# felipeagc/sycl-ray-tracer

Hardware: AMD Instinct MI355X
Metric: Mrays/s (higher is better)
Workload: dtype f32

## Files before the change

include/rt_mi355x.h:

```cpp
#ifndef RT_MI355X_H
#define RT_MI355X_H

#include <stddef.h>
#include <stdint.h>

#ifdef __cplusplus
extern "C" {
#endif

#define RT_ABI_VERSION 8

typedef enum rt_status {
    RT_OK = 0,
    RT_ERR_INVALID = -1,
    RT_ERR_NO_DEVICE = -2,
    RT_ERR_HIP = -3,
    RT_ERR_OOM = -4,
    RT_ERR_UNSUPPORTED = -5
} rt_status;

#define RT_TEX_SIZE 512u
#define RT_TEX_CHANNELS 4u
#define RT_TEX_MAX_LAYERS 128u

// ... 253 lines not shown
                    int want_device_u8);
int rt_frame_gather_begin(rt_comm* c, rt_renderer* const* renderers, int want_f32, int want_u8);
int rt_comm_wait(rt_comm* c, float* rgba_f32, uint8_t* rgba_u8);
int rt_comm_size(const rt_comm* c);
const void* rt_comm_frame_f32(const rt_comm* c);
const void* rt_comm_frame_u8(const rt_comm* c);

int rt_probe_xorshift(int device, uint32_t seed, uint32_t n, float* out, uint32_t* state_out);
int rt_probe_half_roundtrip(int device, uint32_t n, const float* in, float* out,
                            uint16_t* bits_out);
int rt_probe_scatter(rt_scene* scene, uint32_t material, uint32_t n, const float* dir,
                     const float* normal, const float* uv, const uint32_t* seed, uint8_t* ok,
                     float* out_dir, float* out_att, uint32_t* seed_out);

int rt_probe_rounding(int device, uint64_t* mismatches);

const char* rt_last_error(void);
int rt_abi_version(void);
int rt_device_count(void);

#ifdef __cplusplus
}
#endif
#endif
```

sycl-ray-tracer_amd/csrc/rt_device.h:

```cpp
#pragma once
#include <hip/hip_runtime.h>

#include "../../include/rt_mi355x.h"
#include "rt_types.h"

namespace rt {

#define RT_DEV __device__ __forceinline__

struct f3 {
    float x, y, z;
};
RT_DEV f3 mk3(float x, float y, float z) { return f3{x, y, z}; }
RT_DEV f3 operator+(f3 a, f3 b) { return mk3(a.x + b.x, a.y + b.y, a.z + b.z); }
RT_DEV f3 operator-(f3 a, f3 b) { return mk3(a.x - b.x, a.y - b.y, a.z - b.z); }
RT_DEV f3 operator-(f3 a) { return mk3(-a.x, -a.y, -a.z); }
RT_DEV f3 operator*(f3 a, f3 b) { return mk3(a.x * b.x, a.y * b.y, a.z * b.z); }
RT_DEV f3 operator*(float s, f3 a) { return mk3(s * a.x, s * a.y, s * a.z); }
RT_DEV f3 operator*(f3 a, float s) { return mk3(a.x * s, a.y * s, a.z * s); }
RT_DEV float dot3(f3 a, f3 b) { return (a.x * b.x + a.y * b.y) + a.z * b.z; }
RT_DEV f3 cross3(f3 a, f3 b) {
    return mk3(a.y * b.z - a.z * b.y, a.z * b.x - a.x * b.z, a.x * b.y - a.y * b.x);
}
RT_DEV float rcp_rn(float x) {
// ... 6 lines not shown
    return 1.0f / x;
}
RT_DEV float inv_sqrt2(float x) {
    const bool ok = __float_as_uint(x) - 0x0C800000u < 0x73000000u;
    if (__builtin_expect(__builtin_amdgcn_ballot_w64(!ok) == 0ull, 1)) {
        const float r = __builtin_amdgcn_rsqf(x);
        float g = x * r, h = 0.5f * r;
        const float e = __builtin_fmaf(-h, g, 0.5f);
        g = __builtin_fmaf(g, e, g), h = __builtin_fmaf(h, e, h);
        const float s = __builtin_fmaf(__builtin_fmaf(-g, g, x), h, g);
        const float y = __builtin_amdgcn_rcpf(s);
        return __builtin_fmaf(__builtin_fmaf(-s, y, 1.0f), y, y);
    }
    return 1.0f / __builtin_sqrtf(x);
}
RT_DEV f3 normalize3(f3 a) {
    const float inv = inv_sqrt2(dot3(a, a));
    return mk3(a.x * inv, a.y * inv, a.z * inv);
}
RT_DEV float clamp01(float x) { return __builtin_fminf(__builtin_fmaxf(x, 0.0f), 1.0f); }

RT_DEV uint16_t f2h(float f) {
    asm("" : "+v"(f));
    _Float16 h = (_Float16)f;
    return __builtin_bit_cast(uint16_t, h);
}
RT_DEV float h2f(uint16_t b) { return (float)__builtin_bit_cast(_Float16, b); }

RT_DEV float rng_next(uint32_t& a) {
    uint32_t x = a;
    x ^= x << 13;
    x ^= x >> 17;
    x ^= x << 5;
    a = x;
    return (float)x * (1.0f / 4294967296.0f);
}
RT_DEV float rng_range(uint32_t& a, float mn, float mx) { return mn + (mx - mn) * rng_next(a); }
RT_DEV f3 rng_unit_vector(uint32_t& a) {
    float x = rng_range(a, -1.0f, 1.0f);
    float y = rng_range(a, -1.0f, 1.0f);
    float z = rng_range(a, -1.0f, 1.0f);
    return normalize3(mk3(x, y, z));
// ... 170 lines not shown
}
RT_DEV int32_t sel(lmask m, int32_t a, int32_t b) { return (int32_t)sel(m, (uint32_t)a, (uint32_t)b); }

struct TravSigns {
    lmask nx, ny, nz;
};

RT_DEV float ub0(uint32_t w) { return (float)(w & 0xffu); }
RT_DEV float ub1(uint32_t w) { return (float)((w >> 8) & 0xffu); }
RT_DEV float ub2(uint32_t w) { return (float)((w >> 16) & 0xffu); }
RT_DEV float ub3(uint32_t w) { return (float)(w >> 24); }

struct WaveStats {
    uint32_t inner_steps = 0, inner_lanes = 0, leaf_steps = 0, leaf_lanes = 0;
    uint32_t shade_rounds = 0, shade_lanes = 0, live_lane_steps = 0, top_lanes = 0;
};
RT_DEV TravSigns trav_signs(const Trav& T) { return TravSigns{lanes(T.ix < 0.0f), lanes(T.iy < 0.0f), lanes(T.iz < 0.0f)}; }
RT_DEV void trav_inner(const SceneDev& S, Trav& T, const TravStack& stack, const TopTree& top, const TravSigns& sg) {
    const float inf = __builtin_huge_valf();
    float k0, k1, k2, k3;
    u32x4 w0, w1, w2, chw;
    if (T.cur < top.count * 64) {
        const uint32_t o = (uint32_t)T.cur >> 2;
        w0 = *(lds_u32x4*)(size_t)((uint32_t)(size_t)top.w0 + o), w1 = *(lds_u32x4*)(size_t)((uint32_t)(size_t)top.w1 + o);
        w2 = *(lds_u32x4*)(size_t)((uint32_t)(size_t)top.w2 + o), chw = *(lds_u32x4*)(size_t)((uint32_t)(size_t)top.ch + o);
    } else {
        asm volatile("global_load_dwordx4 %0, %4, %5\n\t"
                     "global_load_dwordx4 %1, %4, %5 offset:16\n\t"
                     "global_load_dwordx4 %2, %4, %5 offset:32\n\t"
                     "global_load_dwordx4 %3, %4, %5 offset:48"
// ... 95 lines not shown
}

RT_DEV Hit intersect(const SceneDev& S, f3 o, f3 d, const TravStack& stack, const TopTree& top) {
    Trav T;
    trav_begin(T, o, d, stack);
    const TravSigns sg = trav_signs(T);
    while (trav_step_wave(S, T, stack, top, sg)) {}
    return T.best;
}

RT_DEV bool near_zero3(f3 e) {
    const float s = 1e-8f;
    return (__builtin_fabsf(e.x) < s) && (__builtin_fabsf(e.y) < s) && (__builtin_fabsf(e.z) < s);
}
RT_DEV float length_squared3(f3 v) {
    float l = __builtin_sqrtf(dot3(v, v));
    return l * l;
}
RT_DEV f3 reflect3(f3 v, f3 n) { return v - (2.0f * dot3(v, n)) * n; }
RT_DEV f3 refract3(f3 uv, f3 n, float etai_over_etat) {
    float cos_theta = __builtin_fminf(dot3(-uv, n), 1.0f);
    f3 r_out_perp = etai_over_etat * (uv + cos_theta * n);
    f3 r_out_parallel = (-__builtin_sqrtf(__builtin_fabsf(1.0f - length_squared3(r_out_perp)))) * n;
    return r_out_perp + r_out_parallel;
}
RT_DEV float schlick(float cosine, float ref_idx) {
    float r0 = (1.0f - ref_idx) / (1.0f + ref_idx);
    r0 = r0 * r0;
    float x = 1.0f - cosine;
    float x2 = x * x;
    float x5 = (x2 * x2) * x;
    return r0 + (1.0f - r0) * x5;
}
RT_DEV float unorm8_to_float(uint32_t b) {
    const float x = (float)b, r = 1.0f / 255.0f;
    const float q = x * r;
    return __builtin_fmaf(__builtin_fmaf(-q, 255.0f, x), r, q);
}

RT_DEV bool albedo_is_texture(const MatRec& m) { return (m.type == RT_MAT_DIFFUSE || m.type == RT_MAT_METALLIC) && m.tex_kind != RT_TEX_COLOR; }
RT_DEV uint32_t albedo_fetch(const SceneDev& S, const MatRec& m, float u, float v) {
    float fu = u - __builtin_floorf(u);
    float fv = v - __builtin_floorf(v);
// ... 7 lines not shown
    return mk3(unorm8_to_float(texel & 0xffu), unorm8_to_float((texel >> 8) & 0xffu), unorm8_to_float((texel >> 16) & 0xffu));
}
RT_DEV f3 albedo(const SceneDev& S, const MatRec& m, float u, float v) {
    if (m.tex_kind == RT_TEX_COLOR) return mk3(m.color[0], m.color[1], m.color[2]);
    float fu = u - __builtin_floorf(u);
    float fv = v - __builtin_floorf(v);
    int iu = (int)__builtin_floorf(fu * 512.0f);
    int iv = (int)__builtin_floorf(fv * 512.0f);
    iu = iu < 0 ? 0 : (iu > 511 ? 511 : iu);
    iv = iv < 0 ? 0 : (iv > 511 ? 511 : iv);
    const uint32_t texel = *reinterpret_cast<const uint32_t*>(
        S.tex + (((size_t)m.tex_layer * 512u + (size_t)iv) * 512u + (size_t)iu) * 4u);
    return mk3(unorm8_to_float(texel & 0xffu), unorm8_to_float((texel >> 8) & 0xffu), unorm8_to_float((texel >> 16) & 0xffu));
}

template <bool PRE = false>
RT_DEV bool scatter(const SceneDev& S, const MatRec& m, uint32_t& rng, f3 dir, f3 normal, float u, float v,
                    f3& out_dir, f3& out_att, uint32_t texel = 0) {
    if (m.type == RT_MAT_DIFFUSE || m.type == RT_MAT_METALLIC) {
        const bool diffuse = m.type == RT_MAT_DIFFUSE;
        const f3 unit = rng_unit_vector(rng);
        const f3 reflected = reflect3(dir, normal);
        const f3 base = diffuse ? normal : reflected;
        const f3 offs = diffuse ? unit : m.roughness * unit;
        out_dir = base + offs;
        if (diffuse && near_zero3(dir)) out_dir = normal;
        if (PRE) out_att = m.tex_kind == RT_TEX_COLOR ? mk3(m.color[0], m.color[1], m.color[2]) : albedo_decode(texel);
        else out_att = albedo(S, m, u, v);
        return diffuse ? true : dot3(out_dir, normal) > 0.0f;
    }
    if (m.type == RT_MAT_DIELECTRIC) {
        out_att = mk3(1.0f, 1.0f, 1.0f);
        bool front_face = dot3(dir, normal) < 0.0f;
        f3 n = front_face ? normal : -normal;
        float ratio = front_face ? (1.0f / m.ior) : m.ior;
        f3 unit_direction = normalize3(dir);
        float cos_theta = __builtin_fminf(dot3(-unit_direction, n), 1.0f);
        float sin_theta = __builtin_sqrtf(1.0f - cos_theta * cos_theta);
        bool reflect_it = ratio * sin_theta > 1.0f;
        if (!reflect_it) reflect_it = schlick(cos_theta, ratio) > rng_range(rng, 0.0f, 1.0f);
        out_dir = reflect_it ? reflect3(unit_direction, n) : refract3(unit_direction, n, ratio);
        return true;
    }
    out_dir = mk3(0.0f, 0.0f, 0.0f);
    out_att = mk3(0.0f, 0.0f, 0.0f);
    return false;
}

struct ShadeTables {
    lds_u32x4* nm;
    lds_u32x4* mat;
    uint32_t n_nm, n_mat;
};
RT_DEV void shade_tables_fill(const SceneDev& S, u32x4* nm, u32x4* mat) {
    const u32x4* in = reinterpret_cast<const u32x4*>(S.inst);
    for (uint32_t i = threadIdx.x; i < S.lds_nm * 3u; i += blockDim.x) nm[i] = in[i];
    for (uint32_t i = threadIdx.x; i < S.lds_mats; i += blockDim.x) {
        const u32x4* mp = reinterpret_cast<const u32x4*>(S.mats + i);
        const u32x4 m0 = mp[0], m1 = mp[1], m2 = mp[2];
        u32x4 a, b;
        a.x = m0.x | (m0.y << 8) | (m1.y << 16), a.y = m0.z, a.z = m0.w, a.w = m1.x;
        b.x = m1.z, b.y = m1.w, b.z = m2.x, b.w = m0.x == RT_MAT_DIELECTRIC ? m2.z : m2.y;
        mat[2u * i] = a, mat[2u * i + 1u] = b;
    }
}

#ifdef RT_ROUND_STAMPS
#define RT_STAMP_AFTER(ck, i, VAL)                                                     \
    do {                                                                              \
        if (ck) {                                                                     \
            asm volatile("" ::"v"(VAL));                                              \
            const long long n_ = (long long)__builtin_readcyclecounter();             \
            (ck)[i] += n_ - (ck)[7];                                                  \
            (ck)[7] = n_;                                                             \
        }                                                                             \
    } while (0)
#else
// ... 22 lines not shown
    MatRec mat;
    if (USE_TAB && __builtin_expect(lds, 1)) {
        const uint32_t at = (iw >> kPackedInstBits) * 2u;
        const u32x4 a = tab.mat[at], b = tab.mat[at + 1u];
        mat.type = a.x & 0xffu, mat.tex_kind = (a.x >> 8) & 0xffu, mat.tex_layer = a.x >> 16;
        mat.color[0] = __uint_as_float(a.y), mat.color[1] = __uint_as_float(a.z), mat.color[2] = __uint_as_float(a.w);
        mat.emissive[0] = __uint_as_float(b.x), mat.emissive[1] = __uint_as_float(b.y), mat.emissive[2] = __uint_as_float(b.z);
        mat.roughness = mat.ior = __uint_as_float(b.w);
    } else {
        const InstRec* inst = S.inst + (S.packed_mat ? (iw & kPackedInstMask) : iw);
        const u32x4* mp = reinterpret_cast<const u32x4*>(S.mats + (S.packed_mat ? (iw >> kPackedInstBits) : inst->material));
        const u32x4 m0 = mp[0], m1 = mp[1], m2 = mp[2];
        mat.type = m0.x, mat.tex_kind = m0.y, mat.color[0] = __uint_as_float(m0.z), mat.color[1] = __uint_as_float(m0.w);
        mat.color[2] = __uint_as_float(m1.x), mat.tex_layer = m1.y, mat.emissive[0] = __uint_as_float(m1.z), mat.emissive[1] = __uint_as_float(m1.w);
        mat.emissive[2] = __uint_as_float(m2.x), mat.roughness = __uint_as_float(m2.y), mat.ior = __uint_as_float(m2.z);
    }
    const float bx = h.u, by = h.v;
    const float w = (1.0f - bx) - by;
    const float tu = (w * uv0x + bx * uv1x) + by * uv2x;
    const float tv = (w * uv0y + bx * uv1y) + by * uv2y;
    uint32_t texel;
    {
        float fu = tu - __builtin_floorf(tu);
        float fv = tv - __builtin_floorf(tv);
        int iu = (int)__builtin_floorf(fu * 512.0f);
        int iv = (int)__builtin_floorf(fv * 512.0f);
        iu = iu < 0 ? 0 : (iu > 511 ? 511 : iu);
        iv = iv < 0 ? 0 : (iv > 511 ? 511 : iv);
        const uint8_t* ta = S.tex + (((size_t)mat.tex_layer * 512u + (size_t)iv) * 512u + (size_t)iu) * 4u;
        if (!albedo_is_texture(mat)) ta = reinterpret_cast<const uint8_t*>(sp);
        texel = *reinterpret_cast<const uint32_t*>(ta);
        RT_STAMP_AFTER(ck, 2, ta);
    }
    const bool emits = mat.type == RT_MAT_DIFFUSE || mat.type == RT_MAT_METALLIC;
    rad = rad + (emits ? mk3(mat.emissive[0], mat.emissive[1], mat.emissive[2]) : mk3(0.0f, 0.0f, 0.0f));
    const f3 vn = normalize3((w * n0 + bx * n1) + by * n2);
    float nm[9];
    if (USE_TAB && __builtin_expect(lds, 1)) {
        const uint32_t at = (iw & kPackedInstMask) * 3u;
        const u32x4 a = tab.nm[at], b = tab.nm[at + 1u];
        const uint32_t c = *reinterpret_cast<__attribute__((address_space(3))) const uint32_t*>(tab.nm + at + 2u);
        nm[0] = __uint_as_float(a.x), nm[1] = __uint_as_float(a.y), nm[2] = __uint_as_float(a.z), nm[3] = __uint_as_float(a.w);
        nm[4] = __uint_as_float(b.x), nm[5] = __uint_as_float(b.y), nm[6] = __uint_as_float(b.z), nm[7] = __uint_as_float(b.w);
        nm[8] = __uint_as_float(c);
// ... 8 lines not shown
                     : "=&v"(a), "=&v"(b), "=&v"(c)
                     : "v"(inst)
                     : "memory");
        nm[0] = __uint_as_float(a.x), nm[1] = __uint_as_float(a.y), nm[2] = __uint_as_float(a.z), nm[3] = __uint_as_float(a.w);
        nm[4] = __uint_as_float(b.x), nm[5] = __uint_as_float(b.y), nm[6] = __uint_as_float(b.z), nm[7] = __uint_as_float(b.w);
        nm[8] = __uint_as_float(c);
    }
    const f3 g = mk3((nm[0] * vn.x + nm[3] * vn.y) + nm[6] * vn.z, (nm[1] * vn.x + nm[4] * vn.y) + nm[7] * vn.z,
                     (nm[2] * vn.x + nm[5] * vn.y) + nm[8] * vn.z);
    const f3 normal = normalize3(g);
    RT_STAMP_AFTER(ck, 3, normal.x);
    f3 sdir, satt;
#ifdef RT_SCATTER_PRIO
    __builtin_amdgcn_s_setprio(RT_SCATTER_PRIO);
#endif
    const bool scattered = scatter<true>(S, mat, rng, d, normal, tu, tv, sdir, satt, texel);
    RT_STAMP_AFTER(ck, 4, satt.x);
    if (scattered) {
        org = mk3(org.x + dir.x * h.t, org.y + dir.y * h.t, org.z + dir.z * h.t);
        dir = sdir;
        att = att * satt;
        return false;
    }
    if constexpr (is_no_sink<Sink>::value) result = att * rad;
    else sink(att * rad);
    return true;
}

RT_DEV uint8_t to_unorm8(float c) { return (uint8_t)__builtin_rintf(clamp01(c) * 255.0f); }

#define RT_TRAVERSAL_LDS(BLOCK)                                                                        \
// ... 19 lines not shown
```

sycl-ray-tracer_amd/csrc/rt_frame.hip:

```cpp
#include "rt_internal.h"
#include "rt_kernels.h"



namespace rtlib {

void drop_graph(rt_renderer* r) {
    if (r->graph_exec) (void)hipGraphExecDestroy(r->graph_exec);
    r->graph_exec = nullptr;
}

void free_block_state(rt_renderer* r) {
    if (r->d_blk) (void)hipFree(r->d_blk);
    if (r->d_snap) (void)hipFree(r->d_snap);
    if (r->h_blk) (void)hipHostFree(r->h_blk);
    r->d_blk = nullptr, r->d_snap = nullptr, r->h_blk = nullptr;
    r->blocks_x = r->blocks_y = 0;
    r->h_block_count.clear();
}
size_t blk_words(const rt_renderer* r) { return std::max<size_t>((size_t)r->blocks_x * r->blocks_y, 1); }
int alloc_block_state(rt_renderer* r) {
    free_block_state(r);
    if (!r->d_carry) return RT_OK;
    r->blocks_x = ((uint32_t)r->width + 7u) / 8u, r->blocks_y = ((uint32_t)r->tile.local_rows + 7u) / 8u;
// ... 868 lines not shown
        HIPCHK(hipMemcpy(h, r->d_stats, sizeof(h), hipMemcpyDeviceToHost));
        if (r->kind == RT_RENDERER_MEGAKERNEL && r->stats_level == 1)
            std::fprintf(stderr, "[rt stats] timing-only instantiation: rays %llu | traversal steps %llu | shade/refill rounds %llu\n", rays, h[0], h[4]);
        else
        std::fprintf(stderr,
                     "[rt stats] rays %llu | inner steps %llu (%.1f lanes/step) | leaf steps %llu (%.1f lanes/step) | "
                     "shade/refill rounds %llu (%.1f lanes/round) | live lanes/step %.1f | per ray: %.2f inner (%.2f in the top 341 nodes), %.2f tri\n",
                     rays, h[0], h[0] ? (double)h[1] / h[0] : 0.0, h[2], h[2] ? (double)h[3] / h[2] : 0.0, h[4],
                     h[4] ? (double)h[5] / h[4] : 0.0, (h[0] + h[2]) ? (double)h[6] / (h[0] + h[2]) : 0.0,
                     rays ? (double)h[1] / rays : 0.0, rays ? (double)h[7] / rays : 0.0, rays ? (double)h[3] / rays : 0.0);
        if (h[10])
            std::fprintf(stderr, "[rt stats] waves %llu | cycles per wave: mean %.0f, max %llu | traversal %.1f%%, shading %.1f%% of wave time | "
                         "%.0f cycles per traversal step, %.0f per shade round\n",
                         h[10], (double)h[8] / h[10], h[9], 100.0 * h[11] / h[8], 100.0 * h[12] / h[8],
                         (h[0] + h[2]) ? (double)h[11] / (h[0] + h[2]) : 0.0, h[4] ? (double)h[12] / h[4] : 0.0);
        if (h[10] && h[4] && (h[16] | h[17] | h[18] | h[19] | h[20]))
            std::fprintf(stderr, "[rt stats] shade round, cycles between stamps: record arrived %.0f | material + texel issued %.0f | normal %.0f | scatter + texel arrived %.0f | rest of the round %.0f\n",
                         (double)h[16] / h[4], (double)h[17] / h[4], (double)h[18] / h[4], (double)h[19] / h[4], (double)h[20] / h[4]);
        if (h[10] && h[15] > h[13] && h[14] != ~0ull)
            std::fprintf(stderr, "[rt stats] frame timeline: %.2f ms in all, pixel queue empty after %.2f ms, drain %.2f ms (%.1f%%)\n",
                         (h[15] - h[13]) * 1e-5, (h[14] - h[13]) * 1e-5, (h[15] - h[14]) * 1e-5, 100.0 * (h[15] - h[14]) / (h[15] - h[13]));
    }
    if (stats) *stats = local;
    if (p.req.carry != kCarryNone) {
        r->carry_samples = p.req.carry_total;
        auto& bc = r->h_block_count;
        if (p.req.carry == kCarryStore) std::fill(bc.begin(), bc.end(), spp);
        else if (p.req.carry == kCarryLoadStore) for (auto& c : bc) c += spp;
        else for (uint32_t i = 0; i < p.req.n_blocks; ++i) bc[p.req.blocks[i]] += spp;
        if (!bc.empty()) r->carry_samples = *std::min_element(bc.begin(), bc.end());
// ... 161 lines not shown
```

sycl-ray-tracer_amd/csrc/rt_kernels.h:

```cpp
#pragma once
#include <cstddef>

#include "rt_device.h"
#include "rt_launch.h"

namespace rt {

RT_DEV void queue_store(const QueueDev& q, uint32_t slot, uint32_t id, const RayState& r) {
    q.org_id[slot] = make_float4(r.org.x, r.org.y, r.org.z, __uint_as_float(id));
    q.a[slot] = make_uint2((uint32_t)r.dir[0] | ((uint32_t)r.dir[1] << 16), (uint32_t)r.dir[2] | ((uint32_t)r.att[0] << 16));
    q.b[slot] = make_uint2((uint32_t)r.att[1] | ((uint32_t)r.att[2] << 16), (uint32_t)r.rad[0] | ((uint32_t)r.rad[1] << 16));
    q.c[slot] = r.rad[2];
}
RT_DEV uint32_t queue_load(const QueueDev& q, uint32_t slot, RayState& r) {
    const float4 o = q.org_id[slot];
    const uint2 a = q.a[slot], b = q.b[slot];
    const uint16_t c = q.c[slot];
    r.org = mk3(o.x, o.y, o.z);
    r.dir[0] = (uint16_t)a.x, r.dir[1] = (uint16_t)(a.x >> 16), r.dir[2] = (uint16_t)a.y;
    r.att[0] = (uint16_t)(a.y >> 16), r.att[1] = (uint16_t)b.x, r.att[2] = (uint16_t)(b.x >> 16);
    r.rad[0] = (uint16_t)b.y, r.rad[1] = (uint16_t)(b.y >> 16), r.rad[2] = c;
    return __float_as_uint(o.w);
}

// ... 25 lines not shown

RT_DEV uint32_t wave_sum_u32(uint32_t v) {
#pragma unroll
    for (int off = 32; off > 0; off >>= 1) v += __shfl_down(v, off, 64);
    return v;
}
RT_DEV unsigned long long wave_sum_u64(uint32_t v) {
    return (unsigned long long)wave_sum_u32(v & 0xFFFFu) + ((unsigned long long)wave_sum_u32(v >> 16) << 16);
}

RT_DEV void wave_stats_flush(const WaveStats& ws, unsigned long long* stats_out) {
    atomicAdd(stats_out + 0, (unsigned long long)ws.inner_steps), atomicAdd(stats_out + 1, (unsigned long long)ws.inner_lanes);
    atomicAdd(stats_out + 2, (unsigned long long)ws.leaf_steps), atomicAdd(stats_out + 3, (unsigned long long)ws.leaf_lanes);
    atomicAdd(stats_out + 4, (unsigned long long)ws.shade_rounds), atomicAdd(stats_out + 5, (unsigned long long)ws.shade_lanes);
    atomicAdd(stats_out + 6, (unsigned long long)ws.live_lane_steps), atomicAdd(stats_out + 7, (unsigned long long)ws.top_lanes);
}

template <class F, class I> RT_DEV void pixel_end(const F* sum_r, const F* sum_g, const F* sum_b, float n, I o, float* __restrict__ out_f32, uint8_t* __restrict__ out_u8) {
    const f3 c = mk3(__builtin_sqrtf(*sum_r / n), __builtin_sqrtf(*sum_g / n), __builtin_sqrtf(*sum_b / n));
    if (out_f32) reinterpret_cast<float4*>(out_f32)[o] = make_float4(c.x, c.y, c.z, 1.0f);
    if (out_u8)
        reinterpret_cast<uint32_t*>(out_u8)[o] = (uint32_t)to_unorm8(c.x) | ((uint32_t)to_unorm8(c.y) << 8) | ((uint32_t)to_unorm8(c.z) << 16) | 0xff000000u;
}
RT_DEV uint32_t stream_lane_row(uint32_t r, uint32_t strip_rows, uint32_t n_lanes, uint32_t lane_index) {
    return ((r / strip_rows) * n_lanes + lane_index) * strip_rows + r % strip_rows;
}

#ifndef RT_ROUND_PRIO
#define RT_ROUND_PRIO 0
#endif
constexpr int kMegaUnroll = 3;
#ifndef RT_MEGA_SHADE_PCT
#define RT_MEGA_SHADE_PCT 75
#endif
constexpr uint32_t kMegaShadePct = RT_MEGA_SHADE_PCT;
constexpr uint32_t kMegaRefill = 1;
struct RefillPolicy {
// ... 146 lines not shown
    T.cur = kTravDone;
    constexpr uint32_t kPend = 0x40000000u;
    bool live = false;
    RefillPolicy refill;
    bool exhausted = false;
    uint32_t slice_j = 0;
    auto state_rsrc = [&](const SliceNow& n) {
        return __builtin_amdgcn_make_buffer_rsrc((void*)(((unsigned long long)n.head.y << 32) | n.head.x), 0, (int)((uint32_t)tile.local_rows * (uint32_t)width * 32u), 0x00020000);
    };
    auto take_slot = [&](uint32_t p, uint32_t first) {
        uint32_t t = p >> 6;
        if constexpr (CARRY == 3) t = frame_blocks(frame)[t];
        x = (int)((t % tiles_x) * 8u + (p & 7u));
        const int ly = (int)((t / tiles_x) * 8u + ((p >> 3) & 7u));
        gy = tile_global_row(tile, ly);
        pix = (uint32_t)ly * (uint32_t)width + (uint32_t)x;
        if (x < width && ly < tile.local_rows && gy < height) {
            s = first;
            if (!SLICED || first == 0) {
                depth = 0;
                if constexpr (CARRY >= 2) {
                    const u32x4 c = frame_carry(frame)[pix];
                    rng = c.w;
                    *color_r = __uint_as_float(c.x), *color_g = __uint_as_float(c.y), *color_b = __uint_as_float(c.z);
                    r = camera_ray(frame_camera(frame, width, height), x, gy, rng);
                } else {
                    uint32_t seed_add;
                    const CameraDev cam = frame_camera_and_seed(frame, width, height, seed_add);
                    rng = pixel_seed(x, gy, width, height, seed_mode) + seed_add;
                    *color_r = 0.0f, *color_g = 0.0f, *color_b = 0.0f;
                    r = camera_ray(cam, x, gy, rng);
// ... 67 lines not shown
        if (STATS) {
            ws.shade_rounds++;
            if (STATS >= 2) ws.shade_lanes += (uint32_t)__popcll(__ballot(live && T.cur == kTravDone));
            const long long now = (long long)__builtin_readcyclecounter();
            t_trav += now - t_mark, t_mark = now;
        }
        __builtin_amdgcn_s_setprio(RT_ROUND_PRIO);
#ifdef RT_ROUND_STAMPS
        if (STATS >= 2) ck[7] = (long long)__builtin_readcyclecounter();
#endif
        bool pixel_finished = false;
        {
            const unsigned long long traced = __ballot(live && T.cur == kTravDone && depth < kPend);
            wave_rays += (unsigned long long)__popcll(traced);
            if (SLICED && traced == 0ull && __ballot(live && depth < kPend) == 0ull && slice_wait_count(slice_looks_word(color_r, (lds_f32*)color_lds), frame) && lane == 0) atomicMax(ray_counter + 2, 1ull);
        }
        if (live && T.cur == kTravDone) {
            bool start = false;
            if (SLICED && depth >= kPend) {
                const SliceNow sn = frame_slices(frame);
                const auto rsrc = state_rsrc(sn);
                const uint32_t at = pix * 32u, tag = sn.head.z + s;
                const u32x4 w0 = __builtin_amdgcn_raw_buffer_load_b128(rsrc, (int)at, 0, 16 );
                const u32x4 w1 = __builtin_amdgcn_raw_buffer_load_b128(rsrc, (int)(at + 16u), 0, 16 );
                if ((w0.y == tag && w0.w == tag && w1.y == tag && w1.w == tag) || slice_wait_over(slice_looks_word(color_r, (lds_f32*)color_lds), frame)) {
                    *color_r = __uint_as_float(w0.x), *color_g = __uint_as_float(w0.z), *color_b = __uint_as_float(w1.x);
                    rng = w1.z;
                    start = true;
                }
            } else {
// ... 33 lines not shown
                        __builtin_amdgcn_raw_buffer_store_b128(w1, rsrc, (int)(at + 16u), 0, 16 );
                    } else if (s < spp) {
                        start = true;
                    } else {
                        live = false, pixel_finished = true;
                        float n;
                        if constexpr (CARRY == 3)
                            n = (float)frame_block_count(frame)[(pix / (uint32_t)width >> 3) * tiles_x + ((uint32_t)x >> 3)];
                        else
                            n = (float)(CARRY == 2 ? frame_carry_total(frame) : spp);
                        pixel_end(color_r, color_g, color_b, n, pix, out_f32, out_u8);
                        if constexpr (CARRY != 0) frame_carry(frame)[pix] = carry_word(*color_r, *color_g, *color_b, rng);
                    }
                }
            }
            if (start) {
                depth = 0;
                int cx = x, cy = gy;
                asm volatile("" : "+v"(cx), "+v"(cy));
                r = camera_ray(frame_camera(frame, width, height), cx, cy, rng);
            }
            if (live && depth < kPend) trav_begin(T, r.org, ray_dir(r), stack);
            RT_STAMP_AFTER((STATS >= 2 ? ck : nullptr), 5, T.ox);
        }
        refill.round(pixel_finished);
        if (STATS) t_shade += (long long)__builtin_readcyclecounter() - t_mark;
        __builtin_amdgcn_s_setprio(2);
    }
    if (lane == 0 && wave_rays) atomicAdd(ray_counter, wave_rays);
    if (STATS && lane == 0) {
// ... 834 lines not shown
```

sycl-ray-tracer_amd/csrc/rt_probe_kernels.h:

```cpp
#pragma once
#include "rt_device.h"

namespace rt {

__global__ void __launch_bounds__(256) k_intersect_batch(SceneDev S, uint32_t n, const float* __restrict__ org,
                                                          const float* __restrict__ dir, float* __restrict__ t,
                                                          float* __restrict__ u, float* __restrict__ v,
                                                          uint32_t* __restrict__ tri) {
    RT_TRAVERSAL_LDS(256)
    const uint32_t i = blockIdx.x * 256u + threadIdx.x;
    if (i >= n) return;
    const Hit h = intersect(S, mk3(org[3 * i], org[3 * i + 1], org[3 * i + 2]), mk3(dir[3 * i], dir[3 * i + 1], dir[3 * i + 2]), stack, top);
    t[i] = h.t, u[i] = h.u, v[i] = h.v, tri[i] = h.tri;
}

__global__ void k_probe_xorshift(uint32_t seed, uint32_t n, float* __restrict__ out, uint32_t* __restrict__ state_out) {
    if (threadIdx.x != 0 || blockIdx.x != 0) return;
    uint32_t a = seed;
    for (uint32_t i = 0; i < n; ++i) out[i] = rng_next(a);
    *state_out = a;
}

__global__ void __launch_bounds__(256) k_probe_half(uint32_t n, const float* __restrict__ in, float* __restrict__ out,
                                                     uint16_t* __restrict__ bits) {
// ... 6 lines not shown

__global__ void __launch_bounds__(256) k_probe_rounding(unsigned long long* __restrict__ bad) {
    const uint32_t tid = blockIdx.x * 256u + threadIdx.x, nthreads = gridDim.x * 256u;
    uint32_t b0 = 0, b1 = 0;
    for (unsigned long long i = tid; i < (1ull << 32); i += nthreads) {
        const float x = __uint_as_float((uint32_t)i);
        const float g0 = rcp_rn(x), w0 = 1.0f / x;
        const float g1 = inv_sqrt2(x), w1 = 1.0f / __builtin_sqrtf(x);
        if (__float_as_uint(g0) != __float_as_uint(w0) && !(g0 != g0 && w0 != w0)) b0++;
        if (__float_as_uint(g1) != __float_as_uint(w1) && !(g1 != g1 && w1 != w1)) b1++;
    }
    if (b0) atomicAdd(bad + 0, (unsigned long long)b0);
    if (b1) atomicAdd(bad + 1, (unsigned long long)b1);
}

__global__ void __launch_bounds__(256) k_probe_scatter(SceneDev S, uint32_t material, uint32_t n,
                                                        const float* __restrict__ dir, const float* __restrict__ normal,
                                                        const float* __restrict__ uv, const uint32_t* __restrict__ seed,
                                                        uint8_t* __restrict__ ok, float* __restrict__ out_dir,
                                                        float* __restrict__ out_att, uint32_t* __restrict__ seed_out) {
    const uint32_t i = blockIdx.x * 256u + threadIdx.x;
    if (i >= n) return;
    uint32_t st = seed[i];
    f3 od, oa;
    const bool r = scatter(S, S.mats[material], st, mk3(dir[3 * i], dir[3 * i + 1], dir[3 * i + 2]),
                           mk3(normal[3 * i], normal[3 * i + 1], normal[3 * i + 2]), uv[2 * i], uv[2 * i + 1], od, oa);
    ok[i] = r ? 1 : 0;
    out_dir[3 * i] = od.x, out_dir[3 * i + 1] = od.y, out_dir[3 * i + 2] = od.z;
    out_att[3 * i] = oa.x, out_att[3 * i + 1] = oa.y, out_att[3 * i + 2] = oa.z;
    seed_out[i] = st;
// ... 5 lines not shown
```

sycl-ray-tracer_amd/csrc/rt_probes.hip:

```cpp
#include "rt_internal.h"
#include "rt_probe_kernels.h"

extern "C" {

int rt_intersect_batch(rt_scene* s, uint32_t n, const float* org, const float* dir, float* t, float* u, float* v,
                       uint32_t* tri) {
    if (!s || (n && (!org || !dir || !t || !u || !v || !tri))) return fail(RT_ERR_INVALID, "null argument");
    if (s->device < 0) return fail(RT_ERR_NO_DEVICE, "scene was built host-only (device < 0)");
    if (n == 0) return RT_OK;
    for (uint32_t i = 0; i < n; ++i)
        if (!origin_in_contract_range(s->hs, org + 3 * (size_t)i))
            return fail(RT_ERR_INVALID, "ray " + std::to_string(i) + ": origin more than 100 scene scales outside the scene's bounds (outside the range of the closest-hit contract)");
    HIPCHK(hipSetDevice(s->device));
    DevBuf b_org, b_dir, b_out;
    HIPCHK(b_org.alloc((size_t)n * 12));
    HIPCHK(b_dir.alloc((size_t)n * 12));
    HIPCHK(b_out.alloc((size_t)n * 16));
    float *d_org = b_org.as<float>(), *d_dir = b_dir.as<float>(), *d_out = b_out.as<float>();
    HIPCHK(hipMemcpy(d_org, org, (size_t)n * 12, hipMemcpyHostToDevice));
    HIPCHK(hipMemcpy(d_dir, dir, (size_t)n * 12, hipMemcpyHostToDevice));
    float* d_t = d_out;
    float* d_u = d_out + n;
    float* d_v = d_out + 2 * (size_t)n;
    uint32_t* d_tri = (uint32_t*)(d_out + 3 * (size_t)n);
// ... 45 lines not shown

int rt_probe_rounding(int device, uint64_t* mismatches) {
    if (!mismatches) return fail(RT_ERR_INVALID, "bad arguments");
    int rc = device_ok(device);
    if (rc != RT_OK) return rc;
    DevBuf b;
    HIPCHK(b.alloc(16));
    HIPCHK(hipMemset(b.p, 0, 16));
    hipLaunchKernelGGL(k_probe_rounding, dim3(4096), dim3(256), 0, 0, b.as<unsigned long long>());
    HIPCHK(hipGetLastError());
    HIPCHK(hipDeviceSynchronize());
    HIPCHK(hipMemcpy(mismatches, b.p, 16, hipMemcpyDeviceToHost));
    return RT_OK;
}

int rt_probe_scatter(rt_scene* s, uint32_t material, uint32_t n, const float* dir, const float* normal, const float* uv,
                     const uint32_t* seed, uint8_t* ok, float* out_dir, float* out_att, uint32_t* seed_out) {
    if (!s || !dir || !normal || !uv || !seed || !ok || !out_dir || !out_att || !seed_out || n == 0)
        return fail(RT_ERR_INVALID, "bad arguments");
    if (s->device < 0) return fail(RT_ERR_NO_DEVICE, "scene was built host-only (device < 0)");
    if (material >= s->hs.mats.size()) return fail(RT_ERR_INVALID, "material index out of range");
    HIPCHK(hipSetDevice(s->device));
    DevBuf b_dir, b_nrm, b_uv, b_od, b_oa, b_seed, b_so, b_ok;
    HIPCHK(b_dir.alloc((size_t)n * 12));
    HIPCHK(b_nrm.alloc((size_t)n * 12));
    HIPCHK(b_uv.alloc((size_t)n * 8));
    HIPCHK(b_od.alloc((size_t)n * 12));
    HIPCHK(b_oa.alloc((size_t)n * 12));
    HIPCHK(b_seed.alloc((size_t)n * 4));
    HIPCHK(b_so.alloc((size_t)n * 4));
// ... 19 lines not shown
```

sycl-ray-tracer_amd/rtamd/abi.py:

```python
from __future__ import annotations

import ctypes as C
import os
from pathlib import Path

PKG_DIR = Path(__file__).resolve().parent.parent
REPO_DIR = PKG_DIR.parent
LIB_PATH = PKG_DIR / "csrc" / "build" / "librt_mi355x.so"

RT_OK = 0
RT_ERR_INVALID, RT_ERR_NO_DEVICE, RT_ERR_HIP, RT_ERR_OOM, RT_ERR_UNSUPPORTED = -1, -2, -3, -4, -5

RT_MAT_NONE, RT_MAT_DIFFUSE, RT_MAT_METALLIC, RT_MAT_DIELECTRIC = 0, 1, 2, 3
RT_TEX_COLOR, RT_TEX_IMAGE = 0, 1
RT_RENDERER_MEGAKERNEL, RT_RENDERER_WAVEFRONT = 0, 1
RT_SEED_DEFAULT, RT_SEED_WAVEFRONT, RT_SEED_MEGAKERNEL = 0, 1, 2
RT_BVH_DEFAULT, RT_BVH_LBVH, RT_BVH_SAH, RT_BVH_LBVH_GPU = 0, 1, 2, 3
RT_BVH_MEDIAN_INTERNAL = 99
RT_SCENE_UPDATABLE = 1
RT_SCENE_KEEP_PREVIOUS = 2
RT_TEX_SIZE = 512
RT_TEX_MAX_LAYERS = 128


# ... 234 lines not shown
    "rt_renderer_tile_f32": (C.c_void_p, [C.c_void_p]),
    "rt_renderer_tile_u8": (C.c_void_p, [C.c_void_p]),
    "rt_frame_gather": (C.c_int, [C.c_void_p, _P(C.c_void_p), _P(C.c_float), _P(C.c_uint8), C.c_int, C.c_int]),
    "rt_frame_gather_begin": (C.c_int, [C.c_void_p, _P(C.c_void_p), C.c_int, C.c_int]),
    "rt_comm_wait": (C.c_int, [C.c_void_p, _P(C.c_float), _P(C.c_uint8)]),
    "rt_comm_size": (C.c_int, [C.c_void_p]),
    "rt_comm_frame_f32": (C.c_void_p, [C.c_void_p]),
    "rt_comm_frame_u8": (C.c_void_p, [C.c_void_p]),
    "rt_probe_xorshift": (C.c_int, [C.c_int, C.c_uint32, C.c_uint32, _P(C.c_float), _P(C.c_uint32)]),
    "rt_probe_half_roundtrip": (C.c_int, [C.c_int, C.c_uint32, _P(C.c_float), _P(C.c_float), _P(C.c_uint16)]),
    "rt_probe_scatter": (C.c_int, [C.c_void_p, C.c_uint32, C.c_uint32, _P(C.c_float), _P(C.c_float),
                                   _P(C.c_float), _P(C.c_uint32), _P(C.c_uint8), _P(C.c_float),
                                   _P(C.c_float), _P(C.c_uint32)]),
    "rt_last_error": (C.c_char_p, []),
    "rt_probe_rounding": (C.c_int, [C.c_int, _P(C.c_uint64)]),
    "rt_abi_version": (C.c_int, []),
    "rt_device_count": (C.c_int, []),
}

_lib = None


class RtError(RuntimeError):
    def __init__(self, status: int, msg: str):
        super().__init__(f"rt_status {status}: {msg}")
        self.status = status


def load_library(path: os.PathLike | None = None) -> C.CDLL:
    global _lib
# ... 68 lines not shown
```

Before: 9867.

## Precompute dielectric constants, use fast-path sqrt, and simplify address arithmetic

Adds sqrt_rn, a correctly rounded square root built on rsq plus Newton refinement, with a wave-uniform fallback. It replaces __builtin_sqrtf in the refraction and dielectric scatter math. Dielectric 1/ior and Schlick r0 values are now precomputed into the material table, so scatter stops doing divisions per hit. Texture and output addresses are formed with shift-or helpers that avoid 64-bit multiplies. It also adds a sqrt exactness probe and glass/camera-round statistics counters; the extra work is limited to the new code paths and any mismatch in sqrt rounding could change images.

```diff
diff --git a/include/rt_mi355x.h b/include/rt_mi355x.h
--- a/include/rt_mi355x.h
+++ b/include/rt_mi355x.h
@@ -291,6 +291,7 @@
                      float* out_dir, float* out_att, uint32_t* seed_out);
 
 int rt_probe_rounding(int device, uint64_t* mismatches);
+int rt_probe_sqrt(int device, uint64_t* mismatches);
 
 const char* rt_last_error(void);
 int rt_abi_version(void);
diff --git a/sycl-ray-tracer_amd/csrc/rt_device.h b/sycl-ray-tracer_amd/csrc/rt_device.h
--- a/sycl-ray-tracer_amd/csrc/rt_device.h
+++ b/sycl-ray-tracer_amd/csrc/rt_device.h
@@ -44,6 +44,17 @@
     }
     return 1.0f / __builtin_sqrtf(x);
 }
+RT_DEV float sqrt_rn(float x) {
+    const bool ok = __float_as_uint(x) - 0x0C800000u < 0x73000000u;
+    if (__builtin_expect(__builtin_amdgcn_ballot_w64(!ok) == 0ull, 1)) {
+        const float r = __builtin_amdgcn_rsqf(x);
+        float g = x * r, h = 0.5f * r;
+        const float e = __builtin_fmaf(-h, g, 0.5f);
+        g = __builtin_fmaf(g, e, g), h = __builtin_fmaf(h, e, h);
+        return __builtin_fmaf(__builtin_fmaf(-g, g, x), h, g);
+    }
+    return __builtin_sqrtf(x);
+}
 RT_DEV f3 normalize3(f3 a) {
     const float inv = inv_sqrt2(dot3(a, a));
     return mk3(a.x * inv, a.y * inv, a.z * inv);
@@ -56,6 +67,13 @@
     return __builtin_bit_cast(uint16_t, h);
 }
 RT_DEV float h2f(uint16_t b) { return (float)__builtin_bit_cast(_Float16, b); }
+
+template <uint32_t SH, class T> RT_DEV const T* at_shl_or(const T* base, uint32_t i, uint32_t low) {
+    uint32_t hi = i >> (32u - SH);
+    asm("" : "+v"(hi));
+    return reinterpret_cast<const T*>(reinterpret_cast<const uint8_t*>(base) + (((unsigned long long)hi << 32) | (unsigned long long)((i << SH) | low)));
+}
+template <uint32_t SH, class T> RT_DEV T* at_shl(T* base, uint32_t i) { return const_cast<T*>(at_shl_or<SH>(const_cast<const T*>(base), i, 0u)); }
 
 RT_DEV float rng_next(uint32_t& a) {
     uint32_t x = a;
@@ -256,6 +274,7 @@
 struct WaveStats {
     uint32_t inner_steps = 0, inner_lanes = 0, leaf_steps = 0, leaf_lanes = 0;
     uint32_t shade_rounds = 0, shade_lanes = 0, live_lane_steps = 0, top_lanes = 0;
+    uint32_t glass_rounds = 0, camera_rounds = 0;
 };
 RT_DEV TravSigns trav_signs(const Trav& T) { return TravSigns{lanes(T.ix < 0.0f), lanes(T.iy < 0.0f), lanes(T.iz < 0.0f)}; }
 RT_DEV void trav_inner(const SceneDev& S, Trav& T, const TravStack& stack, const TopTree& top, const TravSigns& sg) {
@@ -381,19 +400,25 @@
     return (__builtin_fabsf(e.x) < s) && (__builtin_fabsf(e.y) < s) && (__builtin_fabsf(e.z) < s);
 }
 RT_DEV float length_squared3(f3 v) {
-    float l = __builtin_sqrtf(dot3(v, v));
+    float l = sqrt_rn(dot3(v, v));
     return l * l;
 }
 RT_DEV f3 reflect3(f3 v, f3 n) { return v - (2.0f * dot3(v, n)) * n; }
 RT_DEV f3 refract3(f3 uv, f3 n, float etai_over_etat) {
     float cos_theta = __builtin_fminf(dot3(-uv, n), 1.0f);
     f3 r_out_perp = etai_over_etat * (uv + cos_theta * n);
-    f3 r_out_parallel = (-__builtin_sqrtf(__builtin_fabsf(1.0f - length_squared3(r_out_perp)))) * n;
+    f3 r_out_parallel = (-sqrt_rn(__builtin_fabsf(1.0f - length_squared3(r_out_perp)))) * n;
     return r_out_perp + r_out_parallel;
 }
-RT_DEV float schlick(float cosine, float ref_idx) {
-    float r0 = (1.0f - ref_idx) / (1.0f + ref_idx);
-    r0 = r0 * r0;
+RT_DEV float schlick_r0(float ref_idx) {
+    const float r0 = (1.0f - ref_idx) / (1.0f + ref_idx);
+    return r0 * r0;
+}
+RT_DEV void dielectric_consts(float ior, float& inv_ior, float& r0_front, float& r0_back) {
+    inv_ior = 1.0f / ior;
+    r0_front = schlick_r0(inv_ior), r0_back = schlick_r0(ior);
+}
+RT_DEV float schlick(float cosine, float r0) {
     float x = 1.0f - cosine;
     float x2 = x * x;
     float x5 = (x2 * x2) * x;
@@ -431,7 +456,7 @@
     return mk3(unorm8_to_float(texel & 0xffu), unorm8_to_float((texel >> 8) & 0xffu), unorm8_to_float((texel >> 16) & 0xffu));
 }
 
-template <bool PRE = false>
+template <bool PRE = false, bool CONSTS = false>
 RT_DEV bool scatter(const SceneDev& S, const MatRec& m, uint32_t& rng, f3 dir, f3 normal, float u, float v,
                     f3& out_dir, f3& out_att, uint32_t texel = 0) {
     if (m.type == RT_MAT_DIFFUSE || m.type == RT_MAT_METALLIC) {
@@ -450,12 +475,18 @@
         out_att = mk3(1.0f, 1.0f, 1.0f);
         bool front_face = dot3(dir, normal) < 0.0f;
         f3 n = front_face ? normal : -normal;
-        float ratio = front_face ? (1.0f / m.ior) : m.ior;
+        float ratio, r0;
+        if (CONSTS) {
+            ratio = front_face ? m.color[0] : m.ior, r0 = front_face ? m.color[1] : m.color[2];
+        } else {
+            ratio = front_face ? (1.0f / m.ior) : m.ior;
+            r0 = schlick_r0(ratio);
+        }
         f3 unit_direction = normalize3(dir);
         float cos_theta = __builtin_fminf(dot3(-unit_direction, n), 1.0f);
-        float sin_theta = __builtin_sqrtf(1.0f - cos_theta * cos_theta);
+        float sin_theta = sqrt_rn(1.0f - cos_theta * cos_theta);
         bool reflect_it = ratio * sin_theta > 1.0f;
-        if (!reflect_it) reflect_it = schlick(cos_theta, ratio) > rng_range(rng, 0.0f, 1.0f);
+        if (!reflect_it) reflect_it = schlick(cos_theta, r0) > rng_range(rng, 0.0f, 1.0f);
         out_dir = reflect_it ? reflect3(unit_direction, n) : refract3(unit_direction, n, ratio);
         return true;
     }
@@ -478,6 +509,11 @@
         u32x4 a, b;
         a.x = m0.x | (m0.y << 8) | (m1.y << 16), a.y = m0.z, a.z = m0.w, a.w = m1.x;
         b.x = m1.z, b.y = m1.w, b.z = m2.x, b.w = m0.x == RT_MAT_DIELECTRIC ? m2.z : m2.y;
+        if (m0.x == RT_MAT_DIELECTRIC) {
+            float inv, r0_front, r0_back;
+            dielectric_consts(__uint_as_float(m2.z), inv, r0_front, r0_back);
+            a.y = __float_as_uint(inv), a.z = __float_as_uint(r0_front), a.w = __float_as_uint(r0_back);
+        }
         mat[2u * i] = a, mat[2u * i + 1u] = b;
     }
 }
@@ -530,6 +566,7 @@
         mat.type = m0.x, mat.tex_kind = m0.y, mat.color[0] = __uint_as_float(m0.z), mat.color[1] = __uint_as_float(m0.w);
         mat.color[2] = __uint_as_float(m1.x), mat.tex_layer = m1.y, mat.emissive[0] = __uint_as_float(m1.z), mat.emissive[1] = __uint_as_float(m1.w);
         mat.emissive[2] = __uint_as_float(m2.x), mat.roughness = __uint_as_float(m2.y), mat.ior = __uint_as_float(m2.z);
+        if (USE_TAB && mat.type == RT_MAT_DIELECTRIC) dielectric_consts(mat.ior, mat.color[0], mat.color[1], mat.color[2]);
     }
     const float bx = h.u, by = h.v;
     const float w = (1.0f - bx) - by;
@@ -543,7 +580,7 @@
         int iv = (int)__builtin_floorf(fv * 512.0f);
         iu = iu < 0 ? 0 : (iu > 511 ? 511 : iu);
         iv = iv < 0 ? 0 : (iv > 511 ? 511 : iv);
-        const uint8_t* ta = S.tex + (((size_t)mat.tex_layer * 512u + (size_t)iv) * 512u + (size_t)iu) * 4u;
+        const uint8_t* ta = at_shl_or<20>(S.tex, mat.tex_layer, ((uint32_t)iv * 512u + (uint32_t)iu) * 4u);
         if (!albedo_is_texture(mat)) ta = reinterpret_cast<const uint8_t*>(sp);
         texel = *reinterpret_cast<const uint32_t*>(ta);
         RT_STAMP_AFTER(ck, 2, ta);
@@ -582,7 +619,7 @@
 #ifdef RT_SCATTER_PRIO
     __builtin_amdgcn_s_setprio(RT_SCATTER_PRIO);
 #endif
-    const bool scattered = scatter<true>(S, mat, rng, d, normal, tu, tv, sdir, satt, texel);
+    const bool scattered = scatter<true, USE_TAB>(S, mat, rng, d, normal, tu, tv, sdir, satt, texel);
     RT_STAMP_AFTER(ck, 4, satt.x);
     if (scattered) {
         org = mk3(org.x + dir.x * h.t, org.y + dir.y * h.t, org.z + dir.z * h.t);
diff --git a/sycl-ray-tracer_amd/csrc/rt_frame.hip b/sycl-ray-tracer_amd/csrc/rt_frame.hip
--- a/sycl-ray-tracer_amd/csrc/rt_frame.hip
+++ b/sycl-ray-tracer_amd/csrc/rt_frame.hip
@@ -906,6 +906,9 @@
                          "%.0f cycles per traversal step, %.0f per shade round\n",
                          h[10], (double)h[8] / h[10], h[9], 100.0 * h[11] / h[8], 100.0 * h[12] / h[8],
                          (h[0] + h[2]) ? (double)h[11] / (h[0] + h[2]) : 0.0, h[4] ? (double)h[12] / h[4] : 0.0);
+        if (r->kind == RT_RENDERER_MEGAKERNEL && r->stats_level == 2 && h[4])
+            std::fprintf(stderr, "[rt stats] shade rounds with a dielectric hit %llu (%.1f%%) | with a camera ray started %llu (%.1f%%)\n", h[21], 100.0 * h[21] / h[4],
+                         h[22], 100.0 * h[22] / h[4]);
         if (h[10] && h[4] && (h[16] | h[17] | h[18] | h[19] | h[20]))
             std::fprintf(stderr, "[rt stats] shade round, cycles between stamps: record arrived %.0f | material + texel issued %.0f | normal %.0f | scatter + texel arrived %.0f | rest of the round %.0f\n",
                          (double)h[16] / h[4], (double)h[17] / h[4], (double)h[18] / h[4], (double)h[19] / h[4], (double)h[20] / h[4]);
diff --git a/sycl-ray-tracer_amd/csrc/rt_kernels.h b/sycl-ray-tracer_amd/csrc/rt_kernels.h
--- a/sycl-ray-tracer_amd/csrc/rt_kernels.h
+++ b/sycl-ray-tracer_amd/csrc/rt_kernels.h
@@ -63,13 +63,14 @@
     atomicAdd(stats_out + 2, (unsigned long long)ws.leaf_steps), atomicAdd(stats_out + 3, (unsigned long long)ws.leaf_lanes);
     atomicAdd(stats_out + 4, (unsigned long long)ws.shade_rounds), atomicAdd(stats_out + 5, (unsigned long long)ws.shade_lanes);
     atomicAdd(stats_out + 6, (unsigned long long)ws.live_lane_steps), atomicAdd(stats_out + 7, (unsigned long long)ws.top_lanes);
+    if (ws.glass_rounds | ws.camera_rounds) atomicAdd(stats_out + 21, (unsigned long long)ws.glass_rounds), atomicAdd(stats_out + 22, (unsigned long long)ws.camera_rounds);
 }
 
 template <class F, class I> RT_DEV void pixel_end(const F* sum_r, const F* sum_g, const F* sum_b, float n, I o, float* __restrict__ out_f32, uint8_t* __restrict__ out_u8) {
     const f3 c = mk3(__builtin_sqrtf(*sum_r / n), __builtin_sqrtf(*sum_g / n), __builtin_sqrtf(*sum_b / n));
-    if (out_f32) reinterpret_cast<float4*>(out_f32)[o] = make_float4(c.x, c.y, c.z, 1.0f);
+    if (out_f32) *at_shl<4>(reinterpret_cast<float4*>(out_f32), (uint32_t)o) = make_float4(c.x, c.y, c.z, 1.0f);
     if (out_u8)
-        reinterpret_cast<uint32_t*>(out_u8)[o] = (uint32_t)to_unorm8(c.x) | ((uint32_t)to_unorm8(c.y) << 8) | ((uint32_t)to_unorm8(c.z) << 16) | 0xff000000u;
+        *at_shl<2>(reinterpret_cast<uint32_t*>(out_u8), (uint32_t)o) = (uint32_t)to_unorm8(c.x) | ((uint32_t)to_unorm8(c.y) << 8) | ((uint32_t)to_unorm8(c.z) << 16) | 0xff000000u;
 }
 RT_DEV uint32_t stream_lane_row(uint32_t r, uint32_t strip_rows, uint32_t n_lanes, uint32_t lane_index) {
     return ((r / strip_rows) * n_lanes + lane_index) * strip_rows + r % strip_rows;
@@ -246,7 +247,9 @@
         x = (int)((t % tiles_x) * 8u + (p & 7u));
         const int ly = (int)((t / tiles_x) * 8u + ((p >> 3) & 7u));
         gy = tile_global_row(tile, ly);
-        pix = (uint32_t)ly * (uint32_t)width + (uint32_t)x;
+        uint32_t row0 = (uint32_t)ly * (uint32_t)width;
+        asm("" : "+v"(row0));
+        pix = row0 + (uint32_t)x;
         if (x < width && ly < tile.local_rows && gy < height) {
             s = first;
             if (!SLICED || first == 0) {
@@ -344,6 +347,14 @@
             const unsigned long long traced = __ballot(live && T.cur == kTravDone && depth < kPend);
             wave_rays += (unsigned long long)__popcll(traced);
             if (SLICED && traced == 0ull && __ballot(live && depth < kPend) == 0ull && slice_wait_count(slice_looks_word(color_r, (lds_f32*)color_lds), frame) && lane == 0) atomicMax(ray_counter + 2, 1ull);
+        }
+        if (STATS >= 2) {
+            bool glass = false;
+            if (live && T.cur == kTravDone && depth < kPend && T.best.tri != kNoTri) {
+                const uint32_t iw = S.shade[T.best.tri].instance;
+                glass = S.mats[S.packed_mat ? iw >> kPackedInstBits : S.inst[iw].material].type == RT_MAT_DIELECTRIC;
+            }
+            if (__ballot(glass) != 0ull) ws.glass_rounds++;
         }
         if (live && T.cur == kTravDone) {
             bool start = false;
@@ -407,6 +418,7 @@
                     }
                 }
             }
+            if (STATS >= 2 && __builtin_amdgcn_ballot_w64(start) != 0ull) ws.camera_rounds++;
             if (start) {
                 depth = 0;
                 int cx = x, cy = gy;
diff --git a/sycl-ray-tracer_amd/csrc/rt_probe_kernels.h b/sycl-ray-tracer_amd/csrc/rt_probe_kernels.h
--- a/sycl-ray-tracer_amd/csrc/rt_probe_kernels.h
+++ b/sycl-ray-tracer_amd/csrc/rt_probe_kernels.h
@@ -44,6 +44,17 @@
     if (b1) atomicAdd(bad + 1, (unsigned long long)b1);
 }
 
+__global__ void __launch_bounds__(256) k_probe_sqrt(unsigned long long* __restrict__ bad) {
+    const uint32_t tid = blockIdx.x * 256u + threadIdx.x, nthreads = gridDim.x * 256u;
+    uint32_t b0 = 0;
+    for (unsigned long long i = tid; i < (1ull << 32); i += nthreads) {
+        const float x = __uint_as_float((uint32_t)i);
+        const float g = sqrt_rn(x), w = __builtin_sqrtf(x);
+        if (__float_as_uint(g) != __float_as_uint(w) && !(g != g && w != w)) b0++;
+    }
+    if (b0) atomicAdd(bad, (unsigned long long)b0);
+}
+
 __global__ void __launch_bounds__(256) k_probe_scatter(SceneDev S, uint32_t material, uint32_t n,
                                                         const float* __restrict__ dir, const float* __restrict__ normal,
                                                         const float* __restrict__ uv, const uint32_t* __restrict__ seed,
diff --git a/sycl-ray-tracer_amd/csrc/rt_probes.hip b/sycl-ray-tracer_amd/csrc/rt_probes.hip
--- a/sycl-ray-tracer_amd/csrc/rt_probes.hip
+++ b/sycl-ray-tracer_amd/csrc/rt_probes.hip
@@ -83,6 +83,20 @@
     return RT_OK;
 }
 
+int rt_probe_sqrt(int device, uint64_t* mismatches) {
+    if (!mismatches) return fail(RT_ERR_INVALID, "bad arguments");
+    int rc = device_ok(device);
+    if (rc != RT_OK) return rc;
+    DevBuf b;
+    HIPCHK(b.alloc(8));
+    HIPCHK(hipMemset(b.p, 0, 8));
+    hipLaunchKernelGGL(k_probe_sqrt, dim3(4096), dim3(256), 0, 0, b.as<unsigned long long>());
+    HIPCHK(hipGetLastError());
+    HIPCHK(hipDeviceSynchronize());
+    HIPCHK(hipMemcpy(mismatches, b.p, 8, hipMemcpyDeviceToHost));
+    return RT_OK;
+}
+
 int rt_probe_scatter(rt_scene* s, uint32_t material, uint32_t n, const float* dir, const float* normal, const float* uv,
                      const uint32_t* seed, uint8_t* ok, float* out_dir, float* out_att, uint32_t* seed_out) {
     if (!s || !dir || !normal || !uv || !seed || !ok || !out_dir || !out_att || !seed_out || n == 0)
diff --git a/sycl-ray-tracer_amd/rtamd/abi.py b/sycl-ray-tracer_amd/rtamd/abi.py
--- a/sycl-ray-tracer_amd/rtamd/abi.py
+++ b/sycl-ray-tracer_amd/rtamd/abi.py
@@ -272,6 +272,7 @@
                                    _P(C.c_float), _P(C.c_uint32)]),
     "rt_last_error": (C.c_char_p, []),
     "rt_probe_rounding": (C.c_int, [C.c_int, _P(C.c_uint64)]),
+    "rt_probe_sqrt": (C.c_int, [C.c_int, _P(C.c_uint64)]),
     "rt_abi_version": (C.c_int, []),
     "rt_device_count": (C.c_int, []),
 }
```

Result: no change. 9901, median of 6 (+0.3%).
